# Intelligent-Microsystems-Lab/SNNQuantPrune

Measured on NVIDIA B200. Metric: TCJA-SNN inference samples/sec (T=20), higher is better.
Workload: dtype int8

## Files before the change

### snnquantprune_b200/csrc/simt.cu

```cuda
#include <stdlib.h>

#include "common.cuh"

namespace snnqp {

template <bool ATT, int MODE>
__global__ void __launch_bounds__(512, 1)
k_conv3x3_simt(const snnqp_block_params p, const uint8_t *__restrict__ x,
               const float *__restrict__ att, const int8_t *__restrict__ wq,
               const float *__restrict__ scale, const float *__restrict__ bias,
               uint8_t *__restrict__ spikes, float *__restrict__ u_final,
               void *__restrict__ acc_dump, float *__restrict__ y_plain, int32_t *__restrict__ counts) {
  extern __shared__ uint32_t sw[];
  const int Cin = p.Cin, Cout = p.Cout, C4 = Cin / 4;
  const uint32_t *wq32 = reinterpret_cast<const uint32_t *>(wq);
  for (int d = threadIdx.x; d < 9 * Cout * C4; d += blockDim.x) {
    const int c4 = d % C4, o = (d / C4) % Cout, tap = d / (C4 * Cout);
    sw[(tap * C4 + c4) * Cout + o] = wq32[d];
  }
  __syncthreads();

  const int o = threadIdx.x % Cout;
  const int lane_q = threadIdx.x / Cout, nlane = blockDim.x / Cout;
  const int H = p.H, W = p.W, QH = H / 2, QW = W / 2;
// ... 381 lines not shown
        const int t = part + 2 * i;
        if (t < T) {
          const uint4 l = *reinterpret_cast<const uint4 *>(lo4 + (t + j) * C4 + 4 * ci16);
          accl[i] = dp4a_us(l.x, w[0], accl[i]); accl[i] = dp4a_us(l.y, w[1], accl[i]);
          accl[i] = dp4a_us(l.z, w[2], accl[i]); accl[i] = dp4a_us(l.w, w[3], accl[i]);
          if constexpr (HIGH) {
            const uint4 h = *reinterpret_cast<const uint4 *>(hi4 + (t + j) * C4 + 4 * ci16);
            acch[i] = dp4a_us(h.x, w[0], acch[i]); acch[i] = dp4a_us(h.y, w[1], acch[i]);
            acch[i] = dp4a_us(h.z, w[2], acch[i]); acch[i] = dp4a_us(h.w, w[3], acch[i]);
          }
        }
      }
    }
  }
#pragma unroll
  for (int i = 0; i < NT; ++i) {
    const int t = part + 2 * i;
    if (t >= T) continue;
    const int acc_c = accl[i] + (HIGH ? acch[i] * 256 : 0);
    int acc_t = 0;
    for (int j = 0; j < 4; ++j) {
      const int cc = c + j - 1;
      if (cc >= 0 && cc < C)
        for (int ti = 0; ti < T; ++ti) acc_t += cnt[ti * C + cc] * (int)qt[(j * T + ti) * T + t];
    }
    const float to = __fmul_rn((float)acc_t, st);
    const float co = __fmul_rn((float)acc_c, scc);
    const float pr = __fmul_rn(co, to);
    const float a = __fdiv_rn(1.0f, __fadd_rn(1.0f, expf(-pr)));
    att[(int64_t)t * p.att_stride_t + (int64_t)b * p.att_stride_b + c] = a;
  }
}

__global__ void __launch_bounds__(256)
k_tcja_att_mma(const snnqp_block_params p, const int32_t *__restrict__ counts,
               const int8_t *__restrict__ wq_t, const int8_t *__restrict__ wq_c,
               const float *__restrict__ scale_t, const float *__restrict__ scale_c,
               float *__restrict__ att) {
  constexpr int C = 128, C4 = C / 4, SA = C4 + 4, SB = C + 8, ROWS = 36;
  extern __shared__ __align__(16) uint8_t tcja_smem[];
  const int b = blockIdx.x, T = p.T;
  uint32_t *qc4 = reinterpret_cast<uint32_t *>(tcja_smem);
  uint32_t *lo4 = qc4 + 4 * C4 * SB;
  uint32_t *hi4 = lo4 + ROWS * SA;
  int32_t *cnt = reinterpret_cast<int32_t *>(hi4 + ROWS * SA);
  int32_t *tout = cnt + T * C;
  int8_t *qt = reinterpret_cast<int8_t *>(tout + T * C);
  for (int d = threadIdx.x; d < 4 * C4 * (C / 16); d += blockDim.x) {
    const int c16 = d % (C / 16), ci4 = (d / (C / 16)) % C4, j = d / ((C / 16) * C4);
    const int4 *src = reinterpret_cast<const int4 *>(wq_c + ((size_t)j * C + 4 * ci4) * C + 16 * c16);
    const int4 r0 = __ldg(src), r1 = __ldg(src + C / 16), r2 = __ldg(src + 2 * (C / 16)), r3 = __ldg(src + 3 * (C / 16));
    uint4 *dst = reinterpret_cast<uint4 *>(qc4 + (j * C4 + ci4) * SB + 16 * c16);
    auto tr = [](uint32_t a, uint32_t b2, uint32_t c, uint32_t e) {
      const uint32_t t0 = __byte_perm(a, b2, 0x5140), t1 = __byte_perm(c, e, 0x5140);
      const uint32_t t2 = __byte_perm(a, b2, 0x7362), t3 = __byte_perm(c, e, 0x7362);
      return make_uint4(__byte_perm(t0, t1, 0x5410), __byte_perm(t0, t1, 0x7632), __byte_perm(t2, t3, 0x5410),
                        __byte_perm(t2, t3, 0x7632));
    };
    dst[0] = tr((uint32_t)r0.x, (uint32_t)r1.x, (uint32_t)r2.x, (uint32_t)r3.x);
    dst[1] = tr((uint32_t)r0.y, (uint32_t)r1.y, (uint32_t)r2.y, (uint32_t)r3.y);
    dst[2] = tr((uint32_t)r0.z, (uint32_t)r1.z, (uint32_t)r2.z, (uint32_t)r3.z);
    dst[3] = tr((uint32_t)r0.w, (uint32_t)r1.w, (uint32_t)r2.w, (uint32_t)r3.w);
  }
  for (int d = threadIdx.x; d < T * C; d += blockDim.x) cnt[d] = counts[(int64_t)b * T * C + d];
  int any_hi = 0;
  for (int d = threadIdx.x; d < ROWS * C4; d += blockDim.x) {
    const int tt = d / C4 - 1, c4 = d % C4;
    uint32_t l = 0, h = 0;
    if (tt >= 0 && tt < T) {
      const int4 v = *reinterpret_cast<const int4 *>(counts + ((int64_t)b * T + tt) * C + 4 * c4);
      l = (v.x & 255) | ((v.y & 255) << 8) | ((v.z & 255) << 16) | ((uint32_t)(v.w & 255) << 24);
      h = ((v.x >> 8) & 255) | (((v.y >> 8) & 255) << 8) | (((v.z >> 8) & 255) << 16) | ((uint32_t)((v.w >> 8) & 255) << 24);
    }
    lo4[(tt + 1) * SA + c4] = l;
    hi4[(tt + 1) * SA + c4] = h;
    any_hi |= (h != 0);
  }
  for (int d = threadIdx.x; d < 4 * T * T; d += blockDim.x) qt[d] = wq_t[d];
  any_hi = __syncthreads_or(any_hi);
  for (int o = threadIdx.x; o < T * C; o += blockDim.x) {
    const int c = o % C, t = o / C;
    int acc_t = 0;
    for (int j = 0; j < 4; ++j) {
      const int cc = c + j - 1;
      if (cc >= 0 && cc < C)
        for (int ti = 0; ti < T; ++ti) acc_t += cnt[ti * C + cc] * (int)qt[(j * T + ti) * T + t];
    }
    tout[o] = acc_t;
  }
  const int warp = threadIdx.x >> 5, lane = threadIdx.x & 31, g = lane >> 2, q = lane & 3;
  int acc[2][2][4], acch[2][2][4];
#pragma unroll
  for (int m = 0; m < 2; ++m)
#pragma unroll
    for (int n = 0; n < 2; ++n)
#pragma unroll
      for (int e = 0; e < 4; ++e) { acc[m][n][e] = 0; acch[m][n][e] = 0; }
  auto mma = [](int (&d)[4], const uint32_t (&a)[4], uint32_t b0, uint32_t b1) {
    asm volatile("mma.sync.aligned.m16n8k32.row.col.s32.u8.s8.s32 {%0,%1,%2,%3}, {%4,%5,%6,%7}, {%8,%9}, {%0,%1,%2,%3};"
                 : "+r"(d[0]), "+r"(d[1]), "+r"(d[2]), "+r"(d[3])
                 : "r"(a[0]), "r"(a[1]), "r"(a[2]), "r"(a[3]), "r"(b0), "r"(b1));
  };
#pragma unroll
  for (int j = 0; j < 4; ++j) {
#pragma unroll
    for (int ks = 0; ks < 4; ++ks) {
      uint32_t bf[2][2];
#pragma unroll
      for (int n = 0; n < 2; ++n) {
        const int col = 16 * warp + 8 * n + g;
        bf[n][0] = qc4[(j * C4 + ks * 8 + q) * SB + col];
        bf[n][1] = qc4[(j * C4 + ks * 8 + q + 4) * SB + col];
      }
#pragma unroll
      for (int m = 0; m < 2; ++m) {
        const uint32_t *r0 = lo4 + (16 * m + g + j) * SA + ks * 8 + q, *r1 = r0 + 8 * SA;
        const uint32_t a[4] = {r0[0], r1[0], r0[4], r1[4]};
#pragma unroll
        for (int n = 0; n < 2; ++n) mma(acc[m][n], a, bf[n][0], bf[n][1]);
        if (any_hi) {
          const uint32_t *h0 = hi4 + (16 * m + g + j) * SA + ks * 8 + q, *h1 = h0 + 8 * SA;
          const uint32_t ah[4] = {h0[0], h1[0], h0[4], h1[4]};
#pragma unroll
          for (int n = 0; n < 2; ++n) mma(acch[m][n], ah, bf[n][0], bf[n][1]);
        }
      }
    }
  }
  __syncthreads();
  const float st = *scale_t, scc = *scale_c;
#pragma unroll
  for (int m = 0; m < 2; ++m)
#pragma unroll
    for (int n = 0; n < 2; ++n)
#pragma unroll
      for (int e = 0; e < 4; ++e) {
        const int t = 16 * m + g + 8 * (e >> 1), c = 16 * warp + 8 * n + 2 * q + (e & 1);
        if (t >= T) continue;
        const int acc_c = acc[m][n][e] + acch[m][n][e] * 256;
        const float to = __fmul_rn((float)tout[t * C + c], st);
        const float co = __fmul_rn((float)acc_c, scc);
        const float pr = __fmul_rn(co, to);
        const float a = __fdiv_rn(1.0f, __fadd_rn(1.0f, expf(-pr)));
        att[(int64_t)t * p.att_stride_t + (int64_t)b * p.att_stride_b + c] = a;
      }
}

__global__ void k_maxpool2(const snnqp_block_params p, const uint8_t *__restrict__ x,
                           uint8_t *__restrict__ y) {
  const int C4 = p.Cin / 4, Ho = p.H / 2, Wo = p.W / 2;
  const int64_t n = (int64_t)p.T * p.B * Ho * Wo * C4;
  for (int64_t i = blockIdx.x * (int64_t)blockDim.x + threadIdx.x; i < n;
       i += (int64_t)gridDim.x * blockDim.x) {
    const int c4 = (int)(i % C4);
    int64_t r = i / C4;
    const int wo = (int)(r % Wo); r /= Wo;
    const int ho = (int)(r % Ho); r /= Ho;
    const int b = (int)(r % p.B);
    const int t = (int)(r / p.B);
    const uint32_t *xp = reinterpret_cast<const uint32_t *>(x + (int64_t)t * p.x_stride_t + (int64_t)b * p.x_stride_b);
    const int64_t base = ((int64_t)(2 * ho) * p.W + 2 * wo) * C4 + c4;
    const uint32_t a = __ldg(xp + base), b2 = __ldg(xp + base + C4);
    const uint32_t c = __ldg(xp + base + (int64_t)p.W * C4), d = __ldg(xp + base + (int64_t)p.W * C4 + C4);
    const uint32_t m = __vmaxu4(__vmaxu4(a, b2), __vmaxu4(c, d));
    reinterpret_cast<uint32_t *>(y + (int64_t)t * p.y_stride_t + (int64_t)b * p.y_stride_b)[((int64_t)ho * Wo + wo) * C4 + c4] = m;
  }
}

__global__ void k_vote(const uint8_t *__restrict__ s, int T, int B, int N, int group,
                       int64_t stride_t, int64_t stride_b, float *__restrict__ logits) {
  const int G = N / group;
  const int idx = blockIdx.x * blockDim.x + threadIdx.x;
  if (idx >= B * G) return;
  const int b = idx / G, g = idx % G;
  float acc = 0.f;
  for (int j = 0; j < group; ++j) {
    int cnt = 0;
    for (int t = 0; t < T; ++t) cnt += s[(int64_t)t * stride_t + (int64_t)b * stride_b + g * group + j];
// ... 64 lines not shown
  }
#undef SNNQP_LAUNCH_CONV
  SNNQP_POST_LAUNCH("k_conv3x3_simt");
  return SNNQP_OK;
}

int launch_dense_simt(const snnqp_block_params &p, int k_pad, const uint8_t *x, const float *att,
                      const int8_t *wq, const float *scale, const float *bias, uint8_t *spikes,
                      float *u_final, void *acc_dump, cudaStream_t st) {
  dim3 grid((p.Cout + 127) / 128, (p.B + DENSE_DB - 1) / DENSE_DB);
  if (att) {
    const size_t smem = (size_t)DENSE_DB * k_pad * 5;
    SNNQP_CUDA(cudaFuncSetAttribute(k_dense_simt<true>, cudaFuncAttributeMaxDynamicSharedMemorySize, (int)smem));
    k_dense_simt<true><<<grid, 128, smem, st>>>(p, k_pad, x, att, wq, scale, bias, spikes, u_final, acc_dump);
  } else {
    const size_t smem = (size_t)DENSE_DB * k_pad;
    k_dense_simt<false><<<grid, 128, smem, st>>>(p, k_pad, x, att, wq, scale, bias, spikes, u_final, acc_dump);
  }
  SNNQP_POST_LAUNCH("k_dense_simt");
  return SNNQP_OK;
}

int launch_tcja(const snnqp_block_params &p, const uint8_t *spikes, const int8_t *wq_t,
                const int8_t *wq_c, const float *scale_t, const float *scale_c, int32_t *counts,
                float *att, cudaStream_t st) {
  if (spikes) {
    k_tcja_counts<<<p.T * p.B, 256, 0, st>>>(p, spikes, counts);
    SNNQP_POST_LAUNCH("k_tcja_counts");
  }
  static const int tcja_impl = getenv("SNNQP_TCJA_IMPL") ? atoi(getenv("SNNQP_TCJA_IMPL")) : 2;
  const bool fast_ok = p.Cin == 128 && p.T <= 32 && (int64_t)p.H * p.W <= 65535 && !(reinterpret_cast<uintptr_t>(counts) & 15) &&
                       !(reinterpret_cast<uintptr_t>(wq_c) & 15);
  if (fast_ok && tcja_impl == 2) {
    const size_t smem_m = (size_t)4 * 32 * 136 * 4 + (size_t)2 * 36 * 36 * 4 + (size_t)2 * p.T * 128 * sizeof(int32_t) +
                          (size_t)4 * p.T * p.T + 16;
    SNNQP_CUDA(cudaFuncSetAttribute(k_tcja_att_mma, cudaFuncAttributeMaxDynamicSharedMemorySize, (int)smem_m));
    k_tcja_att_mma<<<p.B, 256, smem_m, st>>>(p, counts, wq_t, wq_c, scale_t, scale_c, att);
    SNNQP_POST_LAUNCH("k_tcja_att_mma");
    return SNNQP_OK;
  }
  if (fast_ok && tcja_impl == 1) {
    const size_t smem4 = (size_t)4 * 128 * 128 + (size_t)p.T * 128 * sizeof(int32_t) + (size_t)2 * (p.T + 3) * 32 * 4 +
                         (size_t)4 * p.T * p.T + 16;
    if ((int64_t)p.H * p.W <= 255) {
      SNNQP_CUDA(cudaFuncSetAttribute(k_tcja_att_dp4a<false>, cudaFuncAttributeMaxDynamicSharedMemorySize, (int)smem4));
      k_tcja_att_dp4a<false><<<p.B, 256, smem4, st>>>(p, counts, wq_t, wq_c, scale_t, scale_c, att);
    } else {
      SNNQP_CUDA(cudaFuncSetAttribute(k_tcja_att_dp4a<true>, cudaFuncAttributeMaxDynamicSharedMemorySize, (int)smem4));
      k_tcja_att_dp4a<true><<<p.B, 256, smem4, st>>>(p, counts, wq_t, wq_c, scale_t, scale_c, att);
    }
    SNNQP_POST_LAUNCH("k_tcja_att_dp4a");
    return SNNQP_OK;
  }
  const size_t smem = (size_t)4 * p.Cin * p.Cin + (size_t)p.T * p.Cin * sizeof(int32_t) + (size_t)4 * p.T * p.T + 16;
  SNNQP_CUDA(cudaFuncSetAttribute(k_tcja_att, cudaFuncAttributeMaxDynamicSharedMemorySize, (int)smem));
  k_tcja_att<<<p.B, 256, smem, st>>>(p, counts, wq_t, wq_c, scale_t, scale_c, att);
  SNNQP_POST_LAUNCH("k_tcja_att");
  return SNNQP_OK;
}

int launch_maxpool2(const snnqp_block_params &p, const uint8_t *x, uint8_t *y, cudaStream_t st) {
  const int64_t n = (int64_t)p.T * p.B * (p.H / 2) * (p.W / 2) * (p.Cin / 4);
  int64_t g = (n + 255) / 256;
  const int64_t cap = (int64_t)sm_count() * 16;
  if (g > cap) g = cap;
  k_maxpool2<<<(int)g, 256, 0, st>>>(p, x, y);
  SNNQP_POST_LAUNCH("k_maxpool2");
  return SNNQP_OK;
}

int launch_vote(const uint8_t *s, int T, int B, int N, int group, int64_t stride_t,
// ... 16 lines not shown
```

### snnquantprune_b200/csrc/umma_att.cu

```cuda
#include <mutex>

#include "common.cuh"
#include "ptx.cuh"

namespace snnqp {

namespace {

constexpr int kC = 128;
typedef CUresult (*EncodeTiledFn)(CUtensorMap *, CUtensorMapDataType, cuuint32_t, void *, const cuuint64_t *,
                                  const cuuint64_t *, const cuuint32_t *, const cuuint32_t *, CUtensorMapInterleave,
                                  CUtensorMapSwizzle, CUtensorMapL2promotion, CUtensorMapFloatOOBfill);
EncodeTiledFn get_encode2() {
  static EncodeTiledFn fn = nullptr;
  static std::once_flag once;
  std::call_once(once, [] {
    void *p = nullptr;
    cudaDriverEntryPointQueryResult qres;
    if (cudaGetDriverEntryPoint("cuTensorMapEncodeTiled", &p, cudaEnableDefault, &qres) == cudaSuccess &&
        qres == cudaDriverEntryPointSuccess)
      fn = reinterpret_cast<EncodeTiledFn>(p);
  });
  return fn;
}

__device__ __forceinline__ uint32_t nz_mask4(uint32_t w) { return __vcmpne4(w, 0u); }

namespace ca {
constexpr int W = 8, TH = 8, P = 10, N = 80, NI = 3 * N;
constexpr int kPlaneBytes = 13312;
constexpr int kStageBytes = 3 * kPlaneBytes;
constexpr int kWBytes = 9 * kC * kC, kTapBytes = kC * kC;
constexpr int kEpiWarps = 8, kExpWarps = 4;
constexpr int kThreads = (kEpiWarps + 1 + kExpWarps) * 32;
constexpr int kAccStride = 256;
constexpr int kSmemBytes = kWBytes + 2 * kStageBytes + 3 * kC * 2  + 256 + 1024;
}

struct ConvAttArgs {
  int T, B, H;
  int strips, total_items;
  int64_t x_stride_t, x_stride_b, y_stride_t, y_stride_b, att_stride_t, att_stride_b;
  float tau, v_th, v_reset;
  int pool;
  const uint8_t *x;
  const float *att;
  const float *scale, *bias;
  const uint8_t *slab_nz;
  uint8_t *spikes;
  float *u_final;
  float *acc_dump;
  int32_t *counts;
};

template <bool TAU2>
__global__ void __launch_bounds__(ca::kThreads, 1)
k_conv_att_umma(const __grid_constant__ CUtensorMap tmap_w, const ConvAttArgs a) {
  using namespace ca;
  extern __shared__ uint8_t smem_raw[];
  uint8_t *smem = reinterpret_cast<uint8_t *>((reinterpret_cast<uintptr_t>(smem_raw) + 1023) & ~uintptr_t(1023));
  uint8_t *w_smem = smem;
  uint8_t *stage_smem = smem + kWBytes;
  uint8_t *att_smem = stage_smem + 2 * kStageBytes;
  uint64_t *bars = reinterpret_cast<uint64_t *>(att_smem + 2 * 3 * kC);
  uint64_t *w_full = bars, *in_full = bars + 1, *in_empty = bars + 3, *acc_full = bars + 5, *acc_empty = bars + 7;
  uint32_t *tmem_slot = reinterpret_cast<uint32_t *>(bars + 9);

  const int warp = threadIdx.x >> 5, lane = threadIdx.x & 31;
  for (int i = threadIdx.x; i < 2 * kStageBytes / 16; i += kThreads)
    reinterpret_cast<int4 *>(stage_smem)[i] = make_int4(0, 0, 0, 0);
  ptx::fence_proxy_async();
  if (warp == kEpiWarps && lane == 0) {
    ptx::prefetch_tmap(&tmap_w);
    ptx::mbar_init(w_full, 1);
    for (int i = 0; i < 2; ++i) {
      ptx::mbar_init(in_full + i, kExpWarps);
      ptx::mbar_init(in_empty + i, 1);
      ptx::mbar_init(acc_full + i, 1);
      ptx::mbar_init(acc_empty + i, kEpiWarps);
    }
    ptx::fence_barrier_init();
  }
  if (warp == kEpiWarps) ptx::tmem_alloc<512>(tmem_slot);
  ptx::tc_fence_before();
  __syncthreads();
  ptx::tc_fence_after();
  const uint32_t tmem_base = *tmem_slot;

  if (warp == kEpiWarps) {
    if (ptx::elect_one()) {
      ptx::mbar_expect_tx(w_full, kWBytes);
      for (int tap = 0; tap < 9; ++tap) ptx::tma_load_2d(w_smem + tap * kTapBytes, &tmap_w, w_full, 0, tap * kC);
      uint64_t nz_mask = ~0ull;
      if (a.slab_nz) {
        nz_mask = 0;
        for (int i = 0; i < 36; ++i) nz_mask |= (uint64_t)(a.slab_nz[i] != 0) << i;
        if (nz_mask == 0) nz_mask = 1;
      }
      const uint32_t idesc = ptx::make_idesc_i8(128, NI, true, false);
      const uint32_t w_addr = ptx::smem_u32(w_smem);
      const uint64_t desc_hi = ptx::make_desc_sw128(0, 0);
      const bool dense_path = (nz_mask & 0xFFFFFFFFFull) == 0xFFFFFFFFFull;
      ptx::mbar_wait(w_full, 0);
      uint32_t step = 0;
      for (int item = blockIdx.x; item < a.total_items; item += gridDim.x) {
        for (int t = 0; t < a.T; ++t, ++step) {
          const uint32_t s = step & 1, ph = (step >> 1) & 1;
          ptx::mbar_wait(acc_empty + s, ph ^ 1);
          ptx::mbar_wait(in_full + s, ph);
          ptx::tc_fence_after();
          const uint32_t x_addr = ptx::smem_u32(stage_smem + s * kStageBytes);
          const uint64_t ad0 = desc_hi + (w_addr >> 4);
          const uint32_t d_tmem = tmem_base + s * kAccStride;
          const uint64_t bd0 = desc_hi + (x_addr >> 4);
          if (dense_path) {
#pragma unroll
            for (int tap = 0; tap < 9; ++tap)
#pragma unroll
              for (int k = 0; k < 4; ++k)
                ptx::mma_i8(d_tmem, ad0 + (tap * kTapBytes + k * 32) / 16,
                            bd0 + (3 * ((tap / 3) * P + (tap % 3)) * 128 + k * 32) / 16, idesc, (tap | k) != 0);
          } else {
            uint32_t accumulate = 0;
#pragma unroll 1
            for (int sl = 0; sl < 36; ++sl) {
              if (!((nz_mask >> sl) & 1)) continue;
              const int tap = sl >> 2, k = sl & 3;
              ptx::mma_i8(d_tmem, ad0 + (tap * kTapBytes + k * 32) / 16,
                          bd0 + (3 * ((tap / 3) * P + (tap % 3)) * 128 + k * 32) / 16, idesc, accumulate);
              accumulate = 1;
            }
          }
          ptx::mma_commit(in_empty + s);
          ptx::mma_commit(acc_full + s);
        }
      }
    }
  } else if (warp > kEpiWarps) {
    const int et = threadIdx.x - (kEpiWarps + 1) * 32;
    uint32_t step = 0;
    for (int item = blockIdx.x; item < a.total_items; item += gridDim.x) {
// ... 65 lines not shown
        for (int r = 0; r < 4; ++r) {
          const uint32_t taddr = lane_addr + s * kAccStride + 3 * (r0 + r) * P;
          uint32_t lo[16], hi[8];
          SNNQP_TMEM_LD_X16(taddr, lo);
          SNNQP_TMEM_LD_X8(taddr + 16, hi);
#pragma unroll
          for (int i = 0; i < 16; ++i) acc[r][i] = lo[i];
#pragma unroll
          for (int i = 0; i < 8; ++i) acc[r][16 + i] = hi[i];
        }
        ptx::tc_wait_ld();
        ptx::tc_fence_before();
        __syncwarp();
        if (lane == 0) ptx::mbar_arrive(acc_empty + s);

        uint32_t m[4];
        int nspk = 0;
#pragma unroll
        for (int r = 0; r < 4; ++r) {
          m[r] = 0;
#pragma unroll
          for (int j = 0; j < 8; ++j) {
            const float accf = ptx::att_combine((int32_t)acc[r][3 * j], (int32_t)acc[r][3 * j + 1], (int32_t)acc[r][3 * j + 2]);
            const float v = __fmaf_rn(accf, sc, bi);
            bool sp;
            if constexpr (TAU2) {
              const float un = __fadd_rn(u[r][j], __fmul_rn(__fsub_rn(v, __fsub_rn(u[r][j], a.v_reset)), 0.5f));
              sp = __fsub_rn(un, a.v_th) >= 0.0f;
              u[r][j] = sp ? a.v_reset : un;
            } else {
              u[r][j] = lif_step(u[r][j], v, a.tau, a.v_th, a.v_reset, sp);
            }
            m[r] |= (sp ? 1u : 0u) << j;
            if (a.acc_dump)
              a.acc_dump[((((int64_t)t * a.B + b) * a.H + h0 + r0 + r) * W + j) * kC + c] = accf;
          }
          nspk += __popc(m[r]);
        }
        if (a.counts && nspk) atomicAdd(a.counts + ((int64_t)b * a.T + t) * kC + c, nspk);
        uint8_t *yb = a.spikes + (int64_t)t * a.y_stride_t + (int64_t)b * a.y_stride_b + c;
        if (a.pool) {
#pragma unroll
          for (int pr = 0; pr < 2; ++pr) {
            uint32_t mm = m[2 * pr] | m[2 * pr + 1];
            mm |= mm >> 1;
            const int ho = (h0 + r0 + 2 * pr) >> 1;
#pragma unroll
            for (int pc = 0; pc < 4; ++pc) yb[((int64_t)ho * Wo + pc) * kC] = (mm >> (2 * pc)) & 1u;
          }
        } else {
#pragma unroll
          for (int r = 0; r < 4; ++r)
#pragma unroll
            for (int j = 0; j < 8; ++j) yb[((int64_t)(h0 + r0 + r) * Wo + j) * kC] = (m[r] >> j) & 1u;
        }
      }
      if (a.u_final) {
#pragma unroll
        for (int r = 0; r < 4; ++r)
#pragma unroll
          for (int j = 0; j < 8; ++j) a.u_final[(((int64_t)b * a.H + h0 + r0 + r) * W + j) * kC + c] = u[r][j];
      }
    }
  }
  ptx::tc_fence_before();
  __syncthreads();
  if (warp == kEpiWarps) {
    __syncwarp();
    ptx::tc_fence_after();
    ptx::tmem_dealloc<512>(tmem_base);
  }
}

namespace dn {
constexpr int kEpiWarps = 8, kExpWarps = 4;
constexpr int kThreads = (kEpiWarps + 1 + kExpWarps) * 32;
constexpr int kMaxN = 160;
constexpr int kABytes = 128 * 128;
constexpr int kBPlane = kMaxN * 128;
}

struct DenseArgs {
  int T, B, K, Nout;
  int planes;
  int NB, N;
  int m_tiles, col_tiles, total_items;
  int64_t y_stride_t, y_stride_b, att_stride_t, att_stride_b;
  int att_mod;
  float tau, v_th, v_reset;
  const uint8_t *x;
  const float *att;
  const float *scale, *bias;
  uint8_t *spikes;
  float *u_final;
  void *acc_dump;
};

template <int PLANES, bool TAU2>
__global__ void __launch_bounds__(dn::kThreads, 1)
k_dense_umma(const __grid_constant__ CUtensorMap tmap_w, const DenseArgs a) {
  using namespace dn;
  extern __shared__ uint8_t smem_raw[];
  uint8_t *smem = reinterpret_cast<uint8_t *>((reinterpret_cast<uintptr_t>(smem_raw) + 1023) & ~uintptr_t(1023));
  uint8_t *a_smem = smem;
  uint8_t *b_smem = a_smem + 2 * kABytes;
  uint8_t *att_smem = b_smem + 2 * PLANES * kBPlane;
  uint64_t *bars = reinterpret_cast<uint64_t *>(att_smem + (PLANES == 3 ? 3 * kBPlane : 0));
  uint64_t *a_full = bars, *b_full = bars + 2, *ab_empty = bars + 4, *acc_full = bars + 6, *acc_empty = bars + 7;
// ... 32 lines not shown
        const int item = (int)blockIdx.x + (int)(g / kblocks) * (int)gridDim.x;
        ptx::mbar_wait(ab_empty + s, ph ^ 1);
        ptx::mbar_expect_tx(a_full + s, kABytes);
        ptx::tma_load_2d(a_smem + s * kABytes, &tmap_w, a_full + s, (int)(g % kblocks) * 128, (item % a.m_tiles) * 128);
      };
      if (total_steps) issue_load(0);
      for (int item = blockIdx.x; item < a.total_items; item += gridDim.x, ++it) {
        for (int kb = 0; kb < kblocks; ++kb, ++kstep) {
          const uint32_t s = kstep & 1, ph = (kstep >> 1) & 1;
          if (kstep + 1 < total_steps) issue_load(kstep + 1);
          if (kb == 0) ptx::mbar_wait(acc_empty, (it & 1) ^ 1);
          ptx::mbar_wait(a_full + s, ph);
          ptx::mbar_wait(b_full + s, ph);
          ptx::tc_fence_after();
          const uint32_t aa0 = ptx::smem_u32(a_smem + s * kABytes);
          const uint32_t bb0 = ptx::smem_u32(b_smem + s * PLANES * kBPlane);
#pragma unroll
          for (int pl = 0; pl < PLANES; ++pl)
#pragma unroll
            for (int k = 0; k < 4; ++k)
              ptx::mma_i8(tmem_base + pl * kMaxN, ptx::make_desc_sw128(aa0 + k * 32, 0),
                          ptx::make_desc_sw128(bb0 + pl * kBPlane + k * 32, 0), idesc, (kb | k) != 0);
          ptx::mma_commit(ab_empty + s);
        }
        ptx::mma_commit(acc_full);
      }
    }
  } else if (warp > kEpiWarps) {
    const int et = threadIdx.x - (kEpiWarps + 1) * 32;
    uint32_t kstep = 0;
    for (int item = blockIdx.x; item < a.total_items; item += gridDim.x) {
      const int ct = item / a.m_tiles;
      const int row0 = ct * a.N;
      if (PLANES == 3) {
        ptx::named_bar_sync(1, kExpWarps * 32);
        constexpr int kU = 8;
        for (int i0 = et; i0 < a.N * (kC / 4); i0 += kU * kExpWarps * 32) {
          float4 v[kU];
#pragma unroll
          for (int u = 0; u < kU; ++u) {
            const int i4 = i0 + u * kExpWarps * 32;
            const int row = row0 + (i4 >> 5);
            v[u] = make_float4(0.f, 0.f, 0.f, 0.f);
            if (i4 < a.N * (kC / 4) && row < rows_total) {
              const int b = row / a.T, t = row % a.T;
              v[u] = __ldg(reinterpret_cast<const float4 *>(a.att + (int64_t)t * a.att_stride_t + (int64_t)b * a.att_stride_b) +
                           (i4 & 31));
            }
          }
#pragma unroll
          for (int u = 0; u < kU; ++u) {
            const int i4 = i0 + u * kExpWarps * 32;
            if (i4 >= a.N * (kC / 4)) break;
            const uint32_t f0 = ptx::att_fix24(v[u].x), f1 = ptx::att_fix24(v[u].y), f2 = ptx::att_fix24(v[u].z),
                           f3 = ptx::att_fix24(v[u].w);
            const uint32_t lo01 = __byte_perm(f0, f1, 0x5140), lo23 = __byte_perm(f2, f3, 0x5140);
            const uint32_t hi01 = __byte_perm(f0, f1, 0x7362), hi23 = __byte_perm(f2, f3, 0x7362);
            uint32_t *dst = reinterpret_cast<uint32_t *>(att_smem) + i4;
            dst[0 * (kBPlane / 4)] = __byte_perm(hi01, hi23, 0x5410);
            dst[1 * (kBPlane / 4)] = __byte_perm(lo01, lo23, 0x7632);
            dst[2 * (kBPlane / 4)] = __byte_perm(lo01, lo23, 0x5410);
          }
        }
        ptx::named_bar_sync(1, kExpWarps * 32);
      }
      for (int kb = 0; kb < kblocks; ++kb, ++kstep) {
        const uint32_t s = kstep & 1, ph = (kstep >> 1) & 1;
        constexpr int kMaxCh = (kMaxN * 8 + kExpWarps * 32 - 1) / (kExpWarps * 32);
        int4 svs[kMaxCh];
#pragma unroll
        for (int i = 0; i < kMaxCh; ++i) {
          const int ch = et + i * kExpWarps * 32;
          const int row = row0 + (ch >> 3);
          svs[i] = make_int4(0, 0, 0, 0);
          if (ch < a.N * 8 && row < rows_total)
            svs[i] = __ldg(reinterpret_cast<const int4 *>(a.x + (int64_t)row * a.K + kb * 128 + (ch & 7) * 16));
        }
        ptx::mbar_wait(ab_empty + s, ph ^ 1);
        uint8_t *dst = b_smem + s * PLANES * kBPlane;
#pragma unroll
        for (int i = 0; i < kMaxCh; ++i) {
          const int ch = et + i * kExpWarps * 32;
          if (ch >= a.N * 8) break;
          const int r = ch >> 3, c16 = ch & 7;
          const int4 sv = svs[i];
          const uint32_t off = (uint32_t)(r * 128 + ((c16 ^ (r & 7)) << 4));
          if (PLANES == 1) {
            *reinterpret_cast<int4 *>(dst + off) = sv;
          } else {
            const uint32_t m0 = nz_mask4(sv.x), m1 = nz_mask4(sv.y), m2 = nz_mask4(sv.z), m3 = nz_mask4(sv.w);
#pragma unroll
            for (int pl = 0; pl < 3; ++pl) {
              const int4 av = *reinterpret_cast<const int4 *>(att_smem + pl * kBPlane + r * 128 + c16 * 16);
              int4 o;
              o.x = (int)(m0 & (uint32_t)av.x); o.y = (int)(m1 & (uint32_t)av.y);
              o.z = (int)(m2 & (uint32_t)av.z); o.w = (int)(m3 & (uint32_t)av.w);
              *reinterpret_cast<int4 *>(dst + pl * kBPlane + off) = o;
            }
          }
        }
        ptx::fence_proxy_async();
        __syncwarp();
        if (lane == 0) ptx::mbar_arrive(b_full + s);
      }
    }
  } else {
    const int q = warp & 3, g = warp >> 2;
    const uint32_t lane_addr = tmem_base + ((uint32_t)(q * 32) << 16);
    uint32_t it = 0;
    for (int item = blockIdx.x; item < a.total_items; item += gridDim.x, ++it) {
      const int mt = item % a.m_tiles, ct = item / a.m_tiles;
      const int n = mt * 128 + q * 32 + lane;
      const bool act = n < a.Nout;
      const float sc = act ? a.scale[n] : 0.f, bi = act ? a.bias[n] : 0.f;
      const int half = a.N / 2;
      const int col0 = g * half;
      ptx::mbar_wait(acc_full, it & 1);
      ptx::tc_fence_after();
      float u = 0.f;
      int tcur = 0;
      int b = ct * a.NB + g * (a.NB / 2);
      for (int cc = 0; cc < half; cc += 8) {
        uint32_t acc[PLANES][8];
#pragma unroll
        for (int pl = 0; pl < PLANES; ++pl) {
          const uint32_t taddr = lane_addr + pl * kMaxN + col0 + cc;
          SNNQP_TMEM_LD_X8(taddr, acc[pl]);
        }
        ptx::tc_wait_ld();
#pragma unroll
        for (int j = 0; j < 8; ++j) {
          if (tcur == 0) u = 0.f;
          float f;
          if (PLANES == 3) f = ptx::att_combine((int32_t)acc[0][j], (int32_t)acc[PLANES - 1 > 0 ? 1 : 0][j], (int32_t)acc[PLANES - 1][j]);
          else f = (float)(int32_t)acc[0][j];
          const float v = __fmaf_rn(f, sc, bi);
// ... 61 lines not shown
  *N = *NB * T;
  return true;
}

}

bool umma_conv_att_supported(const snnqp_block_params &p, const float *att) {
  if (!att || p.Cin != kC || p.Cout != kC || p.att_mod != kC) return false;
  if (p.W != ca::W || p.H % ca::TH != 0) return false;
  if (p.x_stride_t % 16 || p.x_stride_b % 16) return false;
  return true;
}

int launch_conv_att_umma(const snnqp_block_params &p, const uint8_t *x, const float *att, const int8_t *wq,
                         const float *scale, const float *bias, uint8_t *spikes, float *u_final, float *acc_dump,
                         int32_t *counts, cudaStream_t st) {
  if ((reinterpret_cast<uintptr_t>(x) & 15) || (reinterpret_cast<uintptr_t>(wq) & 15))
    return invalid("tcgen05 conv-att: x and wq must be 16-byte aligned");
  CUtensorMap tmw;
  if (int rc = encode_weights_2d(&tmw, wq, kC, 9 * kC, "conv-att w")) return rc;
  ConvAttArgs a;
  a.T = p.T; a.B = p.B; a.H = p.H;
  a.strips = p.H / ca::TH;
  a.total_items = p.B * a.strips;
  a.x_stride_t = p.x_stride_t; a.x_stride_b = p.x_stride_b;
  a.y_stride_t = p.y_stride_t; a.y_stride_b = p.y_stride_b;
  a.att_stride_t = p.att_stride_t; a.att_stride_b = p.att_stride_b;
  a.tau = p.tau; a.v_th = p.v_threshold; a.v_reset = p.v_reset;
  a.pool = p.pool;
  a.x = x; a.att = att; a.scale = scale; a.bias = bias;
  a.slab_nz = reinterpret_cast<const uint8_t *>(wq) + ca::kWBytes;
  a.spikes = spikes; a.u_final = u_final; a.acc_dump = acc_dump; a.counts = counts;
  const int grid = a.total_items < sm_count() ? a.total_items : sm_count();
  if (p.tau == 2.0f) {
    SNNQP_CUDA(cudaFuncSetAttribute(k_conv_att_umma<true>, cudaFuncAttributeMaxDynamicSharedMemorySize, ca::kSmemBytes));
    k_conv_att_umma<true><<<grid, ca::kThreads, ca::kSmemBytes, st>>>(tmw, a);
  } else {
    SNNQP_CUDA(cudaFuncSetAttribute(k_conv_att_umma<false>, cudaFuncAttributeMaxDynamicSharedMemorySize, ca::kSmemBytes));
    k_conv_att_umma<false><<<grid, ca::kThreads, ca::kSmemBytes, st>>>(tmw, a);
  }
  SNNQP_POST_LAUNCH("k_conv_att_umma");
  return SNNQP_OK;
}

bool umma_dense_supported(const snnqp_block_params &p, const float *att, int k_pad) {
  int NB, N;
  if (p.Cin % 128 != 0 || k_pad != p.Cin) return false;
  if (!dense_tile(p.T, &NB, &N)) return false;
  if (p.x_stride_t != p.Cin || p.x_stride_b != (int64_t)p.T * p.Cin) return false;
  if (att && p.att_mod != kC) return false;
  if (att && ((reinterpret_cast<uintptr_t>(att) & 15) || (p.att_stride_t & 3) || (p.att_stride_b & 3))) return false;
  return true;
}

int launch_dense_umma(const snnqp_block_params &p, const uint8_t *x, const float *att, const int8_t *wq,
                      const float *scale, const float *bias, uint8_t *spikes, float *u_final, void *acc_dump,
                      cudaStream_t st) {
  if ((reinterpret_cast<uintptr_t>(x) & 15) || (reinterpret_cast<uintptr_t>(wq) & 15))
    return invalid("tcgen05 dense: x and wq must be 16-byte aligned");
  CUtensorMap tmw;
  if (int rc = encode_weights_2d(&tmw, wq, (uint64_t)p.Cin, (uint64_t)p.Cout, "dense w")) return rc;
  DenseArgs a;
  a.T = p.T; a.B = p.B; a.K = p.Cin; a.Nout = p.Cout;
  a.planes = att ? 3 : 1;
  dense_tile(p.T, &a.NB, &a.N);
  a.m_tiles = (p.Cout + 127) / 128;
  a.col_tiles = (p.B + a.NB - 1) / a.NB;
  a.total_items = a.m_tiles * a.col_tiles;
  a.y_stride_t = p.y_stride_t; a.y_stride_b = p.y_stride_b;
  a.att_stride_t = p.att_stride_t; a.att_stride_b = p.att_stride_b;
  a.att_mod = p.att_mod;
  a.tau = p.tau; a.v_th = p.v_threshold; a.v_reset = p.v_reset;
  a.x = x; a.att = att; a.scale = scale; a.bias = bias;
// ... 18 lines not shown
```

Measured before the change: 67930.

## Make TCJA attention persistent with tensor-core temporal conv and prefetching

Replaces the per-sample TCJA attention kernel with a persistent kernel. It computes the temporal convolution with mma.sync instead of scalar loops and prefetches the next sample's counts into registers while the current sample computes. The conv-att UMMA kernel gains compile-time template flags: one removes the runtime acc_dump branch, and a default-on serial mode makes the MMA wait on the other accumulator stage. The dense kernel's expand warps go from 4 to 8 and now prefetch the next K-block of activations. Together these target scalar work, launch overhead and load latency, at the cost of more registers and shared memory.

```diff
diff --git a/snnquantprune_b200/csrc/simt.cu b/snnquantprune_b200/csrc/simt.cu
--- a/snnquantprune_b200/csrc/simt.cu
+++ b/snnquantprune_b200/csrc/simt.cu
@@ -437,20 +437,21 @@
   }
 }
 
-__global__ void __launch_bounds__(256)
-k_tcja_att_mma(const snnqp_block_params p, const int32_t *__restrict__ counts,
-               const int8_t *__restrict__ wq_t, const int8_t *__restrict__ wq_c,
-               const float *__restrict__ scale_t, const float *__restrict__ scale_c,
-               float *__restrict__ att) {
+__global__ void __launch_bounds__(256, 1)
+k_tcja_att_persistent(const snnqp_block_params p, const int32_t *__restrict__ counts,
+                      const int8_t *__restrict__ wq_t, const int8_t *__restrict__ wq_c,
+                      const float *__restrict__ scale_t, const float *__restrict__ scale_c,
+                      float *__restrict__ att) {
   constexpr int C = 128, C4 = C / 4, SA = C4 + 4, SB = C + 8, ROWS = 36;
+  constexpr int ST = 12, CROWS = C + 3;
   extern __shared__ __align__(16) uint8_t tcja_smem[];
-  const int b = blockIdx.x, T = p.T;
+  const int T = p.T;
   uint32_t *qc4 = reinterpret_cast<uint32_t *>(tcja_smem);
   uint32_t *lo4 = qc4 + 4 * C4 * SB;
   uint32_t *hi4 = lo4 + ROWS * SA;
-  int32_t *cnt = reinterpret_cast<int32_t *>(hi4 + ROWS * SA);
-  int32_t *tout = cnt + T * C;
-  int8_t *qt = reinterpret_cast<int8_t *>(tout + T * C);
+  uint32_t *loT = hi4 + ROWS * SA;
+  uint32_t *hiT = loT + CROWS * ST;
+  uint32_t *qa = hiT + CROWS * ST;
   for (int d = threadIdx.x; d < 4 * C4 * (C / 16); d += blockDim.x) {
     const int c16 = d % (C / 16), ci4 = (d / (C / 16)) % C4, j = d / ((C / 16) * C4);
     const int4 *src = reinterpret_cast<const int4 *>(wq_c + ((size_t)j * C + 4 * ci4) * C + 16 * c16);
@@ -467,88 +468,128 @@
     dst[2] = tr((uint32_t)r0.z, (uint32_t)r1.z, (uint32_t)r2.z, (uint32_t)r3.z);
     dst[3] = tr((uint32_t)r0.w, (uint32_t)r1.w, (uint32_t)r2.w, (uint32_t)r3.w);
   }
-  for (int d = threadIdx.x; d < T * C; d += blockDim.x) cnt[d] = counts[(int64_t)b * T * C + d];
-  int any_hi = 0;
-  for (int d = threadIdx.x; d < ROWS * C4; d += blockDim.x) {
-    const int tt = d / C4 - 1, c4 = d % C4;
-    uint32_t l = 0, h = 0;
-    if (tt >= 0 && tt < T) {
-      const int4 v = *reinterpret_cast<const int4 *>(counts + ((int64_t)b * T + tt) * C + 4 * c4);
-      l = (v.x & 255) | ((v.y & 255) << 8) | ((v.z & 255) << 16) | ((uint32_t)(v.w & 255) << 24);
-      h = ((v.x >> 8) & 255) | (((v.y >> 8) & 255) << 8) | (((v.z >> 8) & 255) << 16) | ((uint32_t)((v.w >> 8) & 255) << 24);
-    }
-    lo4[(tt + 1) * SA + c4] = l;
-    hi4[(tt + 1) * SA + c4] = h;
-    any_hi |= (h != 0);
-  }
-  for (int d = threadIdx.x; d < 4 * T * T; d += blockDim.x) qt[d] = wq_t[d];
-  any_hi = __syncthreads_or(any_hi);
-  for (int o = threadIdx.x; o < T * C; o += blockDim.x) {
-    const int c = o % C, t = o / C;
-    int acc_t = 0;
-    for (int j = 0; j < 4; ++j) {
-      const int cc = c + j - 1;
-      if (cc >= 0 && cc < C)
-        for (int ti = 0; ti < T; ++ti) acc_t += cnt[ti * C + cc] * (int)qt[(j * T + ti) * T + t];
-    }
-    tout[o] = acc_t;
-  }
+  for (int d = threadIdx.x; d < 2 * ROWS * SA + 2 * CROWS * ST; d += blockDim.x) lo4[d] = 0;
   const int warp = threadIdx.x >> 5, lane = threadIdx.x & 31, g = lane >> 2, q = lane & 3;
-  int acc[2][2][4], acch[2][2][4];
-#pragma unroll
-  for (int m = 0; m < 2; ++m)
-#pragma unroll
-    for (int n = 0; n < 2; ++n)
-#pragma unroll
-      for (int e = 0; e < 4; ++e) { acc[m][n][e] = 0; acch[m][n][e] = 0; }
-  auto mma = [](int (&d)[4], const uint32_t (&a)[4], uint32_t b0, uint32_t b1) {
+  for (int d = threadIdx.x; d < 4 * 2 * 4 * 32; d += blockDim.x) {
+    const int l = d & 31, f = (d >> 5) & 3, m = (d >> 7) & 1, j = d >> 8;
+    const int tp = 16 * m + (l >> 2) + 8 * (f & 1), ti0 = 4 * (l & 3) + 16 * (f >> 1);
+    uint32_t w = 0;
+    for (int k = 0; k < 4; ++k)
+      if (tp < T && ti0 + k < T) w |= (uint32_t)(uint8_t)__ldg(wq_t + (j * T + ti0 + k) * T + tp) << (8 * k);
+    qa[d] = w;
+  }
+  constexpr int kLd = 32 * C4 / 256;
+  int4 cv[kLd];
+  auto load = [&](int b) {
+#pragma unroll
+    for (int i = 0; i < kLd; ++i) {
+      const int d = threadIdx.x + 256 * i, tt = d & 31, c4 = d >> 5;
+      cv[i] = tt < T ? __ldg(reinterpret_cast<const int4 *>(counts + ((int64_t)b * T + tt) * C) + c4) : make_int4(0, 0, 0, 0);
+    }
+  };
+  auto mma_us = [](int (&d)[4], const uint32_t (&a)[4], uint32_t b0, uint32_t b1) {
     asm volatile("mma.sync.aligned.m16n8k32.row.col.s32.u8.s8.s32 {%0,%1,%2,%3}, {%4,%5,%6,%7}, {%8,%9}, {%0,%1,%2,%3};"
                  : "+r"(d[0]), "+r"(d[1]), "+r"(d[2]), "+r"(d[3])
                  : "r"(a[0]), "r"(a[1]), "r"(a[2]), "r"(a[3]), "r"(b0), "r"(b1));
   };
-#pragma unroll
-  for (int j = 0; j < 4; ++j) {
-#pragma unroll
-    for (int ks = 0; ks < 4; ++ks) {
-      uint32_t bf[2][2];
+  auto mma_su = [](int (&d)[4], const uint32_t (&a)[4], uint32_t b0, uint32_t b1) {
+    asm volatile("mma.sync.aligned.m16n8k32.row.col.s32.s8.u8.s32 {%0,%1,%2,%3}, {%4,%5,%6,%7}, {%8,%9}, {%0,%1,%2,%3};"
+                 : "+r"(d[0]), "+r"(d[1]), "+r"(d[2]), "+r"(d[3])
+                 : "r"(a[0]), "r"(a[1]), "r"(a[2]), "r"(a[3]), "r"(b0), "r"(b1));
+  };
+  const float st = *scale_t, scc = *scale_c;
+  int b = blockIdx.x;
+  load(b);
+  for (; b < p.B; b += gridDim.x) {
+    __syncthreads();
+    int any_hi = 0;
+#pragma unroll
+    for (int i = 0; i < kLd; ++i) {
+      const int d = threadIdx.x + 256 * i, tt = d & 31, c4 = d >> 5;
+      if (tt >= T) continue;
+      const int4 v = cv[i];
+      const uint32_t l = (v.x & 255) | ((v.y & 255) << 8) | ((v.z & 255) << 16) | ((uint32_t)(v.w & 255) << 24);
+      const uint32_t h = ((v.x >> 8) & 255) | (((v.y >> 8) & 255) << 8) | (((v.z >> 8) & 255) << 16) |
+                         ((uint32_t)((v.w >> 8) & 255) << 24);
+      lo4[(tt + 1) * SA + c4] = l;
+      hi4[(tt + 1) * SA + c4] = h;
+      uint8_t *lT = reinterpret_cast<uint8_t *>(loT + (4 * c4 + 1) * ST) + tt;
+      uint8_t *hT = reinterpret_cast<uint8_t *>(hiT + (4 * c4 + 1) * ST) + tt;
+#pragma unroll
+      for (int k = 0; k < 4; ++k) {
+        lT[k * 4 * ST] = (uint8_t)(l >> (8 * k));
+        hT[k * 4 * ST] = (uint8_t)(h >> (8 * k));
+      }
+      any_hi |= (h != 0);
+    }
+    any_hi = __syncthreads_or(any_hi);
+    if (b + (int)gridDim.x < p.B) load(b + gridDim.x);
+    int acc[2][2][4], acch[2][2][4], tac[2][2][4], tach[2][2][4];
+#pragma unroll
+    for (int m = 0; m < 2; ++m)
+#pragma unroll
+      for (int n = 0; n < 2; ++n)
+#pragma unroll
+        for (int e = 0; e < 4; ++e) { acc[m][n][e] = 0; acch[m][n][e] = 0; tac[m][n][e] = 0; tach[m][n][e] = 0; }
+#pragma unroll
+    for (int j = 0; j < 4; ++j) {
+      uint32_t a_t[2][4];
+#pragma unroll
+      for (int m = 0; m < 2; ++m)
+#pragma unroll
+        for (int f = 0; f < 4; ++f) a_t[m][f] = qa[((j * 2 + m) * 4 + f) * 32 + lane];
 #pragma unroll
       for (int n = 0; n < 2; ++n) {
-        const int col = 16 * warp + 8 * n + g;
-        bf[n][0] = qc4[(j * C4 + ks * 8 + q) * SB + col];
-        bf[n][1] = qc4[(j * C4 + ks * 8 + q + 4) * SB + col];
-      }
-#pragma unroll
-      for (int m = 0; m < 2; ++m) {
-        const uint32_t *r0 = lo4 + (16 * m + g + j) * SA + ks * 8 + q, *r1 = r0 + 8 * SA;
-        const uint32_t a[4] = {r0[0], r1[0], r0[4], r1[4]};
-#pragma unroll
-        for (int n = 0; n < 2; ++n) mma(acc[m][n], a, bf[n][0], bf[n][1]);
+        const uint32_t *rl = loT + (16 * warp + 8 * n + g + j) * ST + q;
+        mma_su(tac[0][n], a_t[0], rl[0], rl[4]);
+        mma_su(tac[1][n], a_t[1], rl[0], rl[4]);
         if (any_hi) {
-          const uint32_t *h0 = hi4 + (16 * m + g + j) * SA + ks * 8 + q, *h1 = h0 + 8 * SA;
-          const uint32_t ah[4] = {h0[0], h1[0], h0[4], h1[4]};
-#pragma unroll
-          for (int n = 0; n < 2; ++n) mma(acch[m][n], ah, bf[n][0], bf[n][1]);
-        }
-      }
-    }
-  }
-  __syncthreads();
-  const float st = *scale_t, scc = *scale_c;
-#pragma unroll
-  for (int m = 0; m < 2; ++m)
-#pragma unroll
-    for (int n = 0; n < 2; ++n)
-#pragma unroll
-      for (int e = 0; e < 4; ++e) {
-        const int t = 16 * m + g + 8 * (e >> 1), c = 16 * warp + 8 * n + 2 * q + (e & 1);
-        if (t >= T) continue;
-        const int acc_c = acc[m][n][e] + acch[m][n][e] * 256;
-        const float to = __fmul_rn((float)tout[t * C + c], st);
-        const float co = __fmul_rn((float)acc_c, scc);
-        const float pr = __fmul_rn(co, to);
-        const float a = __fdiv_rn(1.0f, __fadd_rn(1.0f, expf(-pr)));
-        att[(int64_t)t * p.att_stride_t + (int64_t)b * p.att_stride_b + c] = a;
-      }
+          const uint32_t *rh = hiT + (16 * warp + 8 * n + g + j) * ST + q;
+          mma_su(tach[0][n], a_t[0], rh[0], rh[4]);
+          mma_su(tach[1][n], a_t[1], rh[0], rh[4]);
+        }
+      }
+#pragma unroll
+      for (int ks = 0; ks < 4; ++ks) {
+        uint32_t bf[2][2];
+#pragma unroll
+        for (int n = 0; n < 2; ++n) {
+          const int col = 16 * warp + 8 * n + g;
+          bf[n][0] = qc4[(j * C4 + ks * 8 + q) * SB + col];
+          bf[n][1] = qc4[(j * C4 + ks * 8 + q + 4) * SB + col];
+        }
+#pragma unroll
+        for (int m = 0; m < 2; ++m) {
+          const uint32_t *r0 = lo4 + (16 * m + g + j) * SA + ks * 8 + q, *r1 = r0 + 8 * SA;
+          const uint32_t a[4] = {r0[0], r1[0], r0[4], r1[4]};
+#pragma unroll
+          for (int n = 0; n < 2; ++n) mma_us(acc[m][n], a, bf[n][0], bf[n][1]);
+          if (any_hi) {
+            const uint32_t *h0 = hi4 + (16 * m + g + j) * SA + ks * 8 + q, *h1 = h0 + 8 * SA;
+            const uint32_t ah[4] = {h0[0], h1[0], h0[4], h1[4]};
+#pragma unroll
+            for (int n = 0; n < 2; ++n) mma_us(acch[m][n], ah, bf[n][0], bf[n][1]);
+          }
+        }
+      }
+    }
+#pragma unroll
+    for (int m = 0; m < 2; ++m)
+#pragma unroll
+      for (int n = 0; n < 2; ++n)
+#pragma unroll
+        for (int e = 0; e < 4; ++e) {
+          const int t = 16 * m + g + 8 * (e >> 1), c = 16 * warp + 8 * n + 2 * q + (e & 1);
+          if (t >= T) continue;
+          const int acc_c = acc[m][n][e] + acch[m][n][e] * 256;
+          const int acc_t = tac[m][n][e] + tach[m][n][e] * 256;
+          const float to = __fmul_rn((float)acc_t, st);
+          const float co = __fmul_rn((float)acc_c, scc);
+          const float pr = __fmul_rn(co, to);
+          const float a = __fdiv_rn(1.0f, __fadd_rn(1.0f, expf(-pr)));
+          att[(int64_t)t * p.att_stride_t + (int64_t)b * p.att_stride_b + c] = a;
+        }
+  }
 }
 
 __global__ void k_maxpool2(const snnqp_block_params p, const uint8_t *__restrict__ x,
@@ -679,11 +720,11 @@
   const bool fast_ok = p.Cin == 128 && p.T <= 32 && (int64_t)p.H * p.W <= 65535 && !(reinterpret_cast<uintptr_t>(counts) & 15) &&
                        !(reinterpret_cast<uintptr_t>(wq_c) & 15);
   if (fast_ok && tcja_impl == 2) {
-    const size_t smem_m = (size_t)4 * 32 * 136 * 4 + (size_t)2 * 36 * 36 * 4 + (size_t)2 * p.T * 128 * sizeof(int32_t) +
-                          (size_t)4 * p.T * p.T + 16;
-    SNNQP_CUDA(cudaFuncSetAttribute(k_tcja_att_mma, cudaFuncAttributeMaxDynamicSharedMemorySize, (int)smem_m));
-    k_tcja_att_mma<<<p.B, 256, smem_m, st>>>(p, counts, wq_t, wq_c, scale_t, scale_c, att);
-    SNNQP_POST_LAUNCH("k_tcja_att_mma");
+    const size_t smem_m = (size_t)4 * 32 * 136 * 4 + (size_t)2 * 36 * 36 * 4 + (size_t)2 * 131 * 12 * 4 + 4 * 2 * 4 * 32 * 4;
+    const int grid = p.B < sm_count() ? p.B : sm_count();
+    SNNQP_CUDA(cudaFuncSetAttribute(k_tcja_att_persistent, cudaFuncAttributeMaxDynamicSharedMemorySize, (int)smem_m));
+    k_tcja_att_persistent<<<grid, 256, smem_m, st>>>(p, counts, wq_t, wq_c, scale_t, scale_c, att);
+    SNNQP_POST_LAUNCH("k_tcja_att_persistent");
     return SNNQP_OK;
   }
   if (fast_ok && tcja_impl == 1) {
diff --git a/snnquantprune_b200/csrc/umma_att.cu b/snnquantprune_b200/csrc/umma_att.cu
--- a/snnquantprune_b200/csrc/umma_att.cu
+++ b/snnquantprune_b200/csrc/umma_att.cu
@@ -1,3 +1,5 @@
+#include <stdlib.h>
+
 #include <mutex>
 
 #include "common.cuh"
@@ -53,7 +55,7 @@
   int32_t *counts;
 };
 
-template <bool TAU2>
+template <bool TAU2, bool DUMP, bool SERIAL>
 __global__ void __launch_bounds__(ca::kThreads, 1)
 k_conv_att_umma(const __grid_constant__ CUtensorMap tmap_w, const ConvAttArgs a) {
   using namespace ca;
@@ -106,7 +108,11 @@
       for (int item = blockIdx.x; item < a.total_items; item += gridDim.x) {
         for (int t = 0; t < a.T; ++t, ++step) {
           const uint32_t s = step & 1, ph = (step >> 1) & 1;
-          ptx::mbar_wait(acc_empty + s, ph ^ 1);
+          if (SERIAL) {
+            if (step) ptx::mbar_wait(acc_empty + (s ^ 1), ((step - 1) >> 1) & 1);
+          } else {
+            ptx::mbar_wait(acc_empty + s, ph ^ 1);
+          }
           ptx::mbar_wait(in_full + s, ph);
           ptx::tc_fence_after();
           const uint32_t x_addr = ptx::smem_u32(stage_smem + s * kStageBytes);
@@ -238,7 +244,7 @@
               u[r][j] = lif_step(u[r][j], v, a.tau, a.v_th, a.v_reset, sp);
             }
             m[r] |= (sp ? 1u : 0u) << j;
-            if (a.acc_dump)
+            if constexpr (DUMP)
               a.acc_dump[((((int64_t)t * a.B + b) * a.H + h0 + r0 + r) * W + j) * kC + c] = accf;
           }
           nspk += __popc(m[r]);
@@ -279,7 +285,10 @@
 }
 
 namespace dn {
-constexpr int kEpiWarps = 8, kExpWarps = 4;
+#ifndef SNNQP_DENSE_EXP_WARPS
+#define SNNQP_DENSE_EXP_WARPS 8
+#endif
+constexpr int kEpiWarps = 8, kExpWarps = SNNQP_DENSE_EXP_WARPS;
 constexpr int kThreads = (kEpiWarps + 1 + kExpWarps) * 32;
 constexpr int kMaxN = 160;
 constexpr int kABytes = 128 * 128;
@@ -378,6 +387,19 @@
     for (int item = blockIdx.x; item < a.total_items; item += gridDim.x) {
       const int ct = item / a.m_tiles;
       const int row0 = ct * a.N;
+      constexpr int kMaxCh = (kMaxN * 8 + kExpWarps * 32 - 1) / (kExpWarps * 32);
+      auto load_x = [&](int kb, int4 (&v)[kMaxCh]) {
+#pragma unroll
+        for (int i = 0; i < kMaxCh; ++i) {
+          const int ch = et + i * kExpWarps * 32;
+          const int row = row0 + (ch >> 3);
+          v[i] = make_int4(0, 0, 0, 0);
+          if (ch < a.N * 8 && row < rows_total)
+            v[i] = __ldg(reinterpret_cast<const int4 *>(a.x + (int64_t)row * a.K + kb * 128 + (ch & 7) * 16));
+        }
+      };
+      int4 svs[kMaxCh];
+      load_x(0, svs);
       if (PLANES == 3) {
         ptx::named_bar_sync(1, kExpWarps * 32);
         constexpr int kU = 8;
@@ -412,16 +434,8 @@
       }
       for (int kb = 0; kb < kblocks; ++kb, ++kstep) {
         const uint32_t s = kstep & 1, ph = (kstep >> 1) & 1;
-        constexpr int kMaxCh = (kMaxN * 8 + kExpWarps * 32 - 1) / (kExpWarps * 32);
-        int4 svs[kMaxCh];
-#pragma unroll
-        for (int i = 0; i < kMaxCh; ++i) {
-          const int ch = et + i * kExpWarps * 32;
-          const int row = row0 + (ch >> 3);
-          svs[i] = make_int4(0, 0, 0, 0);
-          if (ch < a.N * 8 && row < rows_total)
-            svs[i] = __ldg(reinterpret_cast<const int4 *>(a.x + (int64_t)row * a.K + kb * 128 + (ch & 7) * 16));
-        }
+        int4 nxt[kMaxCh];
+        if (kb + 1 < kblocks) load_x(kb + 1, nxt);
         ptx::mbar_wait(ab_empty + s, ph ^ 1);
         uint8_t *dst = b_smem + s * PLANES * kBPlane;
 #pragma unroll
@@ -448,6 +462,8 @@
         ptx::fence_proxy_async();
         __syncwarp();
         if (lane == 0) ptx::mbar_arrive(b_full + s);
+#pragma unroll
+        for (int i = 0; i < kMaxCh; ++i) svs[i] = nxt[i];
       }
     }
   } else {
@@ -575,13 +591,21 @@
   a.slab_nz = reinterpret_cast<const uint8_t *>(wq) + ca::kWBytes;
   a.spikes = spikes; a.u_final = u_final; a.acc_dump = acc_dump; a.counts = counts;
   const int grid = a.total_items < sm_count() ? a.total_items : sm_count();
-  if (p.tau == 2.0f) {
-    SNNQP_CUDA(cudaFuncSetAttribute(k_conv_att_umma<true>, cudaFuncAttributeMaxDynamicSharedMemorySize, ca::kSmemBytes));
-    k_conv_att_umma<true><<<grid, ca::kThreads, ca::kSmemBytes, st>>>(tmw, a);
+  static const bool serial = !(getenv("SNNQP_CONV5_SERIAL") && !atoi(getenv("SNNQP_CONV5_SERIAL")));
+#define SNNQP_LAUNCH_CONV_ATT(T2, DU, SE)                                                                        \
+  do {                                                                                                     \
+    SNNQP_CUDA(cudaFuncSetAttribute(k_conv_att_umma<T2, DU, SE>, cudaFuncAttributeMaxDynamicSharedMemorySize, \
+                                    ca::kSmemBytes));                                                      \
+    k_conv_att_umma<T2, DU, SE><<<grid, ca::kThreads, ca::kSmemBytes, st>>>(tmw, a);                        \
+  } while (0)
+  if (acc_dump) {
+    if (p.tau == 2.0f) SNNQP_LAUNCH_CONV_ATT(true, true, false); else SNNQP_LAUNCH_CONV_ATT(false, true, false);
+  } else if (serial) {
+    if (p.tau == 2.0f) SNNQP_LAUNCH_CONV_ATT(true, false, true); else SNNQP_LAUNCH_CONV_ATT(false, false, true);
   } else {
-    SNNQP_CUDA(cudaFuncSetAttribute(k_conv_att_umma<false>, cudaFuncAttributeMaxDynamicSharedMemorySize, ca::kSmemBytes));
-    k_conv_att_umma<false><<<grid, ca::kThreads, ca::kSmemBytes, st>>>(tmw, a);
-  }
+    if (p.tau == 2.0f) SNNQP_LAUNCH_CONV_ATT(true, false, false); else SNNQP_LAUNCH_CONV_ATT(false, false, false);
+  }
+#undef SNNQP_LAUNCH_CONV_ATT
   SNNQP_POST_LAUNCH("k_conv_att_umma");
   return SNNQP_OK;
 }
```

Measured after the change: 68800, median of 6. +1.3%, better.
